# reazon-research/ReazonSpeech

Measured on AMD Instinct MI355X. Metric: RTFx (audio-sec/wall-sec), FastConformer-RNNT 619M batch=256, higher is better.
Workload: dtype bf16

## Files before the change

### reazonspeech_amd/csrc/k_gemm_bf16.hip

```cpp
#include <stdlib.h>

#include <atomic>

#include "rs_common.h"

namespace {

struct GemmParams {
    const uint16_t* A; const uint16_t* W; void* out;
    const float* bias; const float* residual; const int32_t* mask_lens;
    int lda, ldw, ldc, M, N, K, flags;
    float alpha;
    int mask_rows_per_step, mask_steps;
    int mask_row0;
    int tiles_m, tiles_n;
    int group_m;
    const float* res_ln_stats;
    const float* res_ln_g;
    const float* res_ln_b;
    uint16_t* out2;
    int ld2;
    int pairs;
    long long* trace;
    int cv_T2, cv_F2;
    unsigned cv_b_bytes, cv_t_bytes, cv_f_bytes;
    unsigned cv_seg_bytes;
    int cv_tps, cv_inv;
    const uint16_t* Wfm;
};

enum { OUT_BF16 = 0, OUT_F32 = 1, OUT_RES = 2, OUT_GLU = 3, OUT_RESLN = 4, OUT_BF16S = 5, OUT_F32S = 6, OUT_RES2 = 7 };

template <int N>
__device__ __forceinline__ void wait_vmcnt() {
    if constexpr (N == 0) asm volatile("s_waitcnt vmcnt(0)" ::: "memory");
    else if constexpr (N == 1) asm volatile("s_waitcnt vmcnt(1)" ::: "memory");
    else if constexpr (N == 2) asm volatile("s_waitcnt vmcnt(2)" ::: "memory");
    else if constexpr (N == 3) asm volatile("s_waitcnt vmcnt(3)" ::: "memory");
    else if constexpr (N == 4) asm volatile("s_waitcnt vmcnt(4)" ::: "memory");
    else if constexpr (N == 5) asm volatile("s_waitcnt vmcnt(5)" ::: "memory");
    else if constexpr (N == 6) asm volatile("s_waitcnt vmcnt(6)" ::: "memory");
    else if constexpr (N == 7) asm volatile("s_waitcnt vmcnt(7)" ::: "memory");
    else if constexpr (N == 8) asm volatile("s_waitcnt vmcnt(8)" ::: "memory");
    else if constexpr (N == 12) asm volatile("s_waitcnt vmcnt(12)" ::: "memory");
    else static_assert(N < 0, "add the vmcnt literal");
}

__device__ __forceinline__ void glds16(unsigned voff, const void* sbase, unsigned lds_dst) {
    asm volatile("s_mov_b32 m0, %2\n\ts_nop 0\n\tglobal_load_lds_dwordx4 %0, %1" :: "v"(voff), "s"(sbase), "s"(lds_dst) : "memory");
}

typedef unsigned u32x4_t __attribute__((ext_vector_type(4)));

__device__ __forceinline__ void gload16(u32x4_t& dst, unsigned voff, const void* sbase) {
    asm volatile("global_load_dwordx4 %0, %1, %2" : "=&v"(dst) : "v"(voff), "s"(sbase) : "memory");
}
__device__ __forceinline__ void breg_fence(u32x4_t (&r)[4]) {
    asm volatile("" : "+v"(r[0]), "+v"(r[1]), "+v"(r[2]), "+v"(r[3]) :: "memory");
}
template <int N>
__device__ __forceinline__ void wait_vmcnt_imm() {
    static_assert(N >= 0 && N < 64, "vmcnt is a 6-bit counter");
    asm volatile("s_waitcnt vmcnt(%0)" :: "n"(N) : "memory");
}

__global__ __launch_bounds__(256) void wfm_shuffle_kernel(const uint16_t* __restrict__ W, int ldw, int N, int K, uint16_t* __restrict__ out) {
    const size_t idx = (size_t)blockIdx.x * 256 + threadIdx.x;
    const size_t total = (size_t)N * K / 8;
    if (idx >= total) return;
    const int l = (int)(idx & 63);
    const size_t f = idx >> 6;
    const int kbs = K / 32;
    const int kb = (int)(f % kbs), nb = (int)(f / kbs);
    reinterpret_cast<uint4*>(out)[idx] = *reinterpret_cast<const uint4*>(W + (size_t)(nb * 16 + (l & 15)) * ldw + kb * 32 + (l >> 4) * 8);
}

__device__ __forceinline__ int swz64(int row) { return (row >> 1) & 7; }

__host__ __device__ inline void xcd_split(int xcount, int pair_mode, int& n_pairs, int& n_singles) {
    if (!pair_mode) { n_pairs = 0; n_singles = xcount; return; }
    const int rem = xcount % 64;
    n_singles = rem <= 32 ? rem : (xcount & 1);
    n_pairs = (xcount - n_singles) / 2;
}

template <int MI, int NI, int OUT_KIND, bool MASK, int PF>
__device__ __forceinline__ void smf16_epilogue(const GemmParams& p, f32x4_t (&acc)[MI][NI], char* scr, int cm0, int cn0,
                                               int wm, int wn, int lane) {
    constexpr bool SWOOSH = OUT_KIND == OUT_BF16S || OUT_KIND == OUT_F32S, RES2 = OUT_KIND == OUT_RES2;
    constexpr int OUT = OUT_KIND == OUT_BF16S ? OUT_BF16 : (OUT_KIND == OUT_F32S ? OUT_F32 : (RES2 ? OUT_RES : OUT_KIND));
    constexpr bool RESLN = OUT == OUT_RESLN, RES = OUT == OUT_RES || RESLN, out_f32 = OUT == OUT_F32 || RES, GLU = OUT == OUT_GLU, rowmask = MASK;
    constexpr int TM = MI * 16, TN = NI * 16;
    constexpr unsigned OOB = 0xfffffff0u;
    const int frow = lane & 15, fch = lane >> 4;
    const int flags = p.flags;
    const bool has_bias = flags & RS_GEMM_BIAS, relu = flags & RS_GEMM_RELU, silu = flags & RS_GEMM_SILU;
    const bool swl = SWOOSH && (flags & RS_GEMM_SWOOSHL), swr = SWOOSH && (flags & RS_GEMM_SWOOSHR);
    const float alpha = p.alpha;
    const size_t out_bytes = (size_t)p.M * p.ldc * (out_f32 ? 4 : 2);
    const auto out_rsrc = __builtin_amdgcn_make_buffer_rsrc(p.out, 0, (int)out_bytes, 0x00020000);
    const auto res_rsrc = __builtin_amdgcn_make_buffer_rsrc(const_cast<float*>(RES ? p.residual : (const float*)p.out), 0,
                                                            (int)out_bytes, 0x00020000);
    const auto bias_rsrc = __builtin_amdgcn_make_buffer_rsrc(const_cast<float*>(has_bias ? p.bias : (const float*)p.out), 0,
                                                             has_bias ? p.N * 4 : 0, 0x00020000);
    const int wrow0 = cm0 + wm * TM, wcol0 = cn0 + wn * TN;
    float4 bias_r[NI];
#pragma unroll
    for (int jj = 0; jj < NI; ++jj) {
        const int n = wcol0 + jj * 16 + 4 * fch;
        const u32x4_t b = __builtin_amdgcn_raw_buffer_load_b128(bias_rsrc, (unsigned)n * 4u, 0, 0);
        bias_r[jj] = __builtin_bit_cast(float4, b);
    }
    auto finish = [&](int i, int jj) -> float4 {
        float4 v = make_float4(acc[i][jj][0] + bias_r[jj].x, acc[i][jj][1] + bias_r[jj].y, acc[i][jj][2] + bias_r[jj].z,
                               acc[i][jj][3] + bias_r[jj].w);
        if (relu) { v.x = fmaxf(v.x, 0.f); v.y = fmaxf(v.y, 0.f); v.z = fmaxf(v.z, 0.f); v.w = fmaxf(v.w, 0.f); }
        if (silu) { v.x = silu_f(v.x); v.y = silu_f(v.y); v.z = silu_f(v.z); v.w = silu_f(v.w); }
        if constexpr (SWOOSH) {
            if (swl) { v.x = swoosh_l_f(v.x); v.y = swoosh_l_f(v.y); v.z = swoosh_l_f(v.z); v.w = swoosh_l_f(v.w); }
            if (swr) { v.x = swoosh_r_f(v.x); v.y = swoosh_r_f(v.y); v.z = swoosh_r_f(v.z); v.w = swoosh_r_f(v.w); }
        }
        v.x *= alpha; v.y *= alpha; v.z *= alpha; v.w *= alpha;
        return v;
    };
    auto row_keep = [&](int m) -> bool {
        if (!rowmask || m >= p.M) return true;
        const int step = (m + p.mask_row0) / p.mask_rows_per_step;
        const int b = step / p.mask_steps;
        return step - b * p.mask_steps < p.mask_lens[b];
    };
    if constexpr (GLU) {
        static_assert(NI == 4, "GLU epilogue: 64-column wave tiles");
        const int rr4 = lane >> 2, cc = lane & 3;
        const int ocol0 = wcol0 >> 1;
#pragma unroll
        for (int c = 0; c < MI / 2; ++c) {
#pragma unroll
            for (int il = 0; il < 2; ++il)
#pragma unroll
                for (int jj = 0; jj < 2; ++jj) {
                    const float4 a = finish(2 * c + il, jj), g = finish(2 * c + il, jj + 2);
                    const int row = il * 16 + frow;
                    const int piece = (jj * 2 + (fch >> 1)) ^ ((row >> 1) & 3);
                    *reinterpret_cast<u16x4_t*>(scr + row * 64 + piece * 16 + (fch & 1) * 8) =
                        pack_bf16x4(a.x * sigmoid_f(g.x), a.y * sigmoid_f(g.y), a.z * sigmoid_f(g.z), a.w * sigmoid_f(g.w));
                }
#pragma unroll
            for (int sgm = 0; sgm < 2; ++sgm) {
                const int row = sgm * 16 + rr4;
                u32x4_t d = *reinterpret_cast<const u32x4_t*>(scr + row * 64 + ((cc ^ ((row >> 1) & 3)) * 16));
                const int m = wrow0 + c * 32 + row, n = ocol0 + cc * 8;
                if (!row_keep(m)) d = (u32x4_t){0u, 0u, 0u, 0u};
                const unsigned off = (m < p.M && 2 * n < p.N) ? ((unsigned)m * (unsigned)p.ldc + (unsigned)n) * 2u : OOB;
                __builtin_amdgcn_raw_buffer_store_b128(d, out_rsrc, off, 0, 0);
            }
        }
    } else if constexpr (!out_f32) {
        const int rr8 = lane >> 3, cc = lane & 7;
#pragma unroll
        for (int c = 0; c < MI / 2; ++c) {
#pragma unroll
            for (int il = 0; il < 2; ++il)
#pragma unroll
                for (int jj = 0; jj < NI; ++jj) {
                    const float4 v = finish(2 * c + il, jj);
                    const int row = il * 16 + frow;
                    const int piece = (jj * 2 + (fch >> 1)) ^ (row & 7);
                    *reinterpret_cast<u16x4_t*>(scr + row * 128 + piece * 16 + (fch & 1) * 8) = pack_bf16x4(v.x, v.y, v.z, v.w);
                }
#pragma unroll
            for (int sgm = 0; sgm < 4; ++sgm) {
                const int row = sgm * 8 + rr8;
                u32x4_t d = *reinterpret_cast<const u32x4_t*>(scr + row * 128 + ((cc ^ (row & 7)) * 16));
                const int m = wrow0 + c * 32 + row, n = wcol0 + cc * 8;
                if (!row_keep(m)) d = (u32x4_t){0u, 0u, 0u, 0u};
                const unsigned off = (m < p.M && n < p.N) ? ((unsigned)m * (unsigned)p.ldc + (unsigned)n) * 2u : OOB;
                __builtin_amdgcn_raw_buffer_store_b128(d, out_rsrc, off, 0, 0);
            }
        }
    } else {
        const int rr4 = lane >> 4, cc = lane & 15;
        constexpr int PFE = (RESLN && MI >= 8 && PF > 1) ? PF - 1 : PF;
        constexpr int NPF = RES ? (PFE < 1 ? 1 : (PFE > MI ? MI : PFE)) : 1;
        u32x4_t rvq[NPF][4];
        float2 stq[NPF][4];
        float4 ln_g = make_float4(0.f, 0.f, 0.f, 0.f), ln_b = ln_g;
        const auto st_rsrc = __builtin_amdgcn_make_buffer_rsrc(const_cast<float*>(RESLN ? p.res_ln_stats : (const float*)p.out), 0,
                                                               RESLN ? p.M * 8 : 0, 0x00020000);
        if constexpr (RESLN) {
            const int n = wcol0 + cc * 4;
            if (n < p.N) {
                ln_g = *reinterpret_cast<const float4*>(p.res_ln_g + n);
                ln_b = *reinterpret_cast<const float4*>(p.res_ln_b + n);
            }
        }
        auto load_res = [&](int i, u32x4_t (&rv)[4], float2 (&st)[4]) {
#pragma unroll
            for (int sgm = 0; sgm < 4; ++sgm) {
                const int m = wrow0 + i * 16 + sgm * 4 + rr4, n = wcol0 + cc * 4;
                const unsigned off = (m < p.M && n < p.N) ? ((unsigned)m * (unsigned)p.ldc + (unsigned)n) * 4u : OOB;
                rv[sgm] = __builtin_amdgcn_raw_buffer_load_b128(res_rsrc, off, 0, 0);
                if constexpr (RESLN)
                    st[sgm] = __builtin_bit_cast(float2, __builtin_amdgcn_raw_buffer_load_b64(st_rsrc, m < p.M ? (unsigned)m * 8u : OOB, 0, 0));
            }
        };
        if constexpr (RES) {
#pragma unroll
            for (int d = 0; d < NPF; ++d) load_res(d, rvq[d], stq[d]);
            __builtin_amdgcn_sched_barrier(0);
        }
#pragma unroll
        for (int i = 0; i < MI; ++i) {
            u32x4_t rv[4];
            float2 st[4];
            if constexpr (RES) {
#pragma unroll
                for (int sgm = 0; sgm < 4; ++sgm) { rv[sgm] = rvq[i % NPF][sgm]; st[sgm] = stq[i % NPF][sgm]; }
            }
#pragma unroll
            for (int jj = 0; jj < NI; ++jj) {
                const float4 v = finish(i, jj);
                const int piece = (jj * 4 + fch) ^ frow;
                *reinterpret_cast<float4*>(scr + frow * 256 + piece * 16) = v;
            }
#pragma unroll
            for (int sgm = 0; sgm < 4; ++sgm) {
                const int row = sgm * 4 + rr4;
                float4 v = *reinterpret_cast<const float4*>(scr + row * 256 + ((cc ^ row) * 16));
                if constexpr (RES) {
                    float4 r = __builtin_bit_cast(float4, rv[sgm]);
                    if constexpr (RESLN) {
                        const float mean = st[sgm].x, rstd = st[sgm].y;
                        r.x = fmaf((r.x - mean) * rstd, ln_g.x, ln_b.x); r.y = fmaf((r.y - mean) * rstd, ln_g.y, ln_b.y);
                        r.z = fmaf((r.z - mean) * rstd, ln_g.z, ln_b.z); r.w = fmaf((r.w - mean) * rstd, ln_g.w, ln_b.w);
                    }
                    v.x += r.x; v.y += r.y; v.z += r.z; v.w += r.w;
                }
                const int m = wrow0 + i * 16 + row, n = wcol0 + cc * 4;
                if (!row_keep(m)) v = make_float4(0.f, 0.f, 0.f, 0.f);
                const unsigned off = (m < p.M && n < p.N) ? ((unsigned)m * (unsigned)p.ldc + (unsigned)n) * 4u : OOB;
                __builtin_amdgcn_raw_buffer_store_b128(__builtin_bit_cast(u32x4_t, v), out_rsrc, off, 0, 0);
                if constexpr (RES2) {
                    if (m < p.M && n < p.N) *reinterpret_cast<u16x4_t*>(p.out2 + (size_t)m * p.ld2 + n) = pack_bf16x4(v.x, v.y, v.z, v.w);
                }
            }
            if constexpr (RES) {
                if (i + NPF < MI) load_res(i + NPF, rvq[i % NPF], stq[i % NPF]);
            }
            __builtin_amdgcn_sched_barrier(0);
        }
    }
}

template <int BM, int OUT, bool MASK, int EPF, bool TRACE, bool CONVA = false, bool BREG = false>
__global__ __launch_bounds__(512, 2) void gemm_smf16_kernel(GemmParams p) {
    constexpr int BN = 256, WN = 4, NWAVES = 8;
    constexpr int TM = BM / 2, TN = BN / WN, MI = TM / 16, NI = TN / 16;
    constexpr int SLOT = 32768, NSLOT = 5;
    constexpr int LA = BM / 8 / NWAVES, LB = BN / 8 / NWAVES;
    constexpr int NPH = 2;
    static_assert((BM == 256 || BM == 192 || BM == 128 || BM == 64) && LB == 4 && (MI % 2) == 0 && BM * 128 <= SLOT, "tile heights");
    constexpr int A_BYTES = BM * 128, STAGE = A_BYTES + SLOT;
    constexpr bool R3 = 3 * STAGE <= NSLOT * SLOT;
    static_assert(!BREG || (!R3 && !TRACE && NI == 4), "BREG: split-ring tiles (256 / 192 rows) only");
    long long tr_t0 = 0, tr_t1 = 0, tr_t2 = 0, tr_w0 = 0, tr_stall = 0;
    if constexpr (TRACE) { tr_t0 = __builtin_readcyclecounter(); tr_w0 = (long long)wall_clock64(); }
    extern __shared__ __attribute__((aligned(16))) char smem[];
    const int tid = threadIdx.x, lane = tid & 63;
    const int wave = __builtin_amdgcn_readfirstlane(tid >> 6);
    const int wm = wave / WN, wn = wave % WN;
    const int frow = lane & 15, fch = lane >> 4;
    const unsigned lds0 = (unsigned)(size_t)(__attribute__((address_space(3))) char*)smem;

    const int nwg = p.tiles_m * p.tiles_n;
    const int bid = blockIdx.x;
    const int xcd = bid & 7, xslot = bid >> 3;
    const int q8 = nwg >> 3, rr = nwg & 7;
    const int xbase = xcd < rr ? xcd * (q8 + 1) : rr * (q8 + 1) + (xcd - rr) * q8;
    const int xcount = xcd < rr ? q8 + 1 : q8;
    int n_pairs, n_singles;
    xcd_split(xcount, p.pairs, n_pairs, n_singles);
    if (xslot >= n_pairs + n_singles) return;
    const int first_tile = xslot < n_pairs ? 2 * xslot : 2 * n_pairs + (xslot - n_pairs);
    const int n_my = xslot < n_pairs ? 2 : 1;
    const int nk = p.K / 64;
    const bool carry = p.pairs == 2 && nk >= 2;
    const int dr = lane >> 3, dpc = lane & 7;
    auto tile_origin = [&](int j, int& m0, int& n0) {
        const int wg = xbase + first_tile + j;
        const int per_group = p.group_m * p.tiles_n;
        const int g = wg / per_group, r = wg - g * per_group;
        const int left = p.tiles_m - g * p.group_m;
        const int gm = left < p.group_m ? left : p.group_m;
        const int tile_n = r / gm;
        m0 = (g * p.group_m + (r - tile_n * gm)) * BM;
        n0 = tile_n * BN;
    };
    auto lane_offsets = [&](int m0, int n0, unsigned (&o)[LA + LB]) {
#pragma unroll
        for (int j = 0; j < LA; ++j) {
            const int row = (wave + NWAVES * j) * 8 + dr;
            int gr = m0 + row;
            gr = gr < p.M ? gr : p.M - 1;
            if constexpr (CONVA) {
                const int bt = gr / p.cv_F2, f2 = gr - bt * p.cv_F2;
                const int b = bt / p.cv_T2, t2 = bt - b * p.cv_T2;
                o[j] = (unsigned)b * p.cv_b_bytes + (unsigned)t2 * p.cv_t_bytes + (unsigned)f2 * p.cv_f_bytes + (unsigned)((dpc ^ swz64(row)) * 16);
            } else {
                o[j] = (unsigned)gr * (unsigned)(p.lda * 2) + (unsigned)((dpc ^ swz64(row)) * 16);
            }
        }
        if constexpr (BREG) return;
#pragma unroll
        for (int j = 0; j < LB; ++j) {
            const int row = (wave * LB + j) * 8 + dr;
            int gr = n0 + row;
            gr = gr < p.N ? gr : p.N - 1;
            o[LA + j] = (unsigned)gr * (unsigned)(p.ldw * 2) + (unsigned)((dpc ^ swz64(row)) * 16);
        }
    };
    u32x4_t breg[2][4];
    const unsigned bvoff = (unsigned)lane * 16u;
    auto bfrag_base = [&](int n0_, int kb) -> const char* {
        const int nb = (n0_ >> 4) + wn * NI;
        const size_t off = ((size_t)nb * (size_t)(p.K >> 5) + (size_t)kb) << 10;
        return reinterpret_cast<const char*>(p.Wfm) + off;
    };
    auto bload = [&](int set, int n0_, int kb) {
        const char* b0 = bfrag_base(n0_, kb);
        const size_t jstride = (size_t)(p.K >> 5) << 10;
#pragma unroll
        for (int jj = 0; jj < 4; ++jj) gload16(breg[set][jj], bvoff, b0 + jj * jstride);
    };
    auto frag = [&](const char* part, int row, int chunk) -> bf16x8_t {
        return *reinterpret_cast<const bf16x8_t*>(part + row * 128 + ((chunk ^ swz64(row)) << 4));
    };
    auto wrap = [](int v) { return v >= NSLOT ? v - NSLOT : v; };

    int m0, n0;
    unsigned off[LA + LB], offn[LA + LB];
    tile_origin(0, m0, n0);
    lane_offsets(m0, n0, off);
    int sa = 0;
  for (int it = 0; it < n_my; ++it) {
    const bool has_next = carry && it + 1 < n_my;
    int m1 = m0, n1 = n0;
    if (has_next) { tile_origin(it + 1, m1, n1); lane_offsets(m1, n1, offn); }
    auto dma_a = [&](int j, int k, int dst) {
        const bool nx = k >= nk;
        const int kt = nx ? k - nk : k;
        size_t kbytes = (size_t)kt * 128;
        if constexpr (CONVA) {
            const int sg = (kt * p.cv_inv) >> 16;
            kbytes = (size_t)sg * p.cv_seg_bytes + (size_t)(kt - sg * p.cv_tps) * 128;
        }
        glds16(nx ? offn[j] : off[j], reinterpret_cast<const char*>(p.A) + kbytes, lds0 + dst + (wave + NWAVES * j) * 1024);
    };
    auto dma_b = [&](int j, int k, int dst) {
        if constexpr (BREG) return;
        const bool nx = k >= nk;
        glds16(nx ? offn[LA + j] : off[LA + j], reinterpret_cast<const char*>(p.W) + (size_t)(nx ? k - nk : k) * 128,
               lds0 + dst + (wave * LB + j) * 1024);
    };
    if constexpr (BREG) {
        if (it == 0 || !carry) {
            sa = 0;
#pragma unroll
            for (int j = 0; j < LA; ++j) dma_a(j, 0, 0);
            if (nk > 1) {
#pragma unroll
                for (int j = 0; j < LA; ++j) dma_a(j, 1, 2 * SLOT);
            }
            bload(0, n0, 0);
            bload(1, n0, 1);
            if (nk > 1) wait_vmcnt_imm<LA + 2 * NI>();
            else wait_vmcnt_imm<2 * NI>();
            __builtin_amdgcn_s_barrier();
        } else {
            bload(0, n0, 0);
            bload(1, n0, 1);
        }
    } else
    if (it == 0 || !carry) {
        sa = 0;
#pragma unroll
        for (int j = 0; j < LA; ++j) dma_a(j, 0, 0);
#pragma unroll
        for (int j = 0; j < LB; ++j) dma_b(j, 0, R3 ? A_BYTES : SLOT);
        if (nk > 1) {
#pragma unroll
            for (int j = 0; j < LA; ++j) dma_a(j, 1, R3 ? STAGE : 2 * SLOT);
            if constexpr (R3) {
#pragma unroll
                for (int j = 0; j < LB; ++j) dma_b(j, 1, STAGE + A_BYTES);
                wait_vmcnt<LA + LB>();
            } else if (wm == 1) {
#pragma unroll
                for (int j = 0; j < LB; ++j) dma_b(j, 1, 3 * SLOT);
                wait_vmcnt<LA + LB>();
            } else {
                wait_vmcnt<LA>();
            }
        } else {
            wait_vmcnt<0>();
        }
        __builtin_amdgcn_s_barrier();
    }
    if (wm == 1) __builtin_amdgcn_s_barrier();
    if constexpr (TRACE) tr_t1 = __builtin_readcyclecounter();

    f32x4_t acc[MI][NI];
#pragma unroll
    for (int i = 0; i < MI; ++i)
#pragma unroll
        for (int jj = 0; jj < NI; ++jj)
#pragma unroll
            for (int e = 0; e < 4; ++e) acc[i][jj][e] = 0.0f;

    for (int t = 0; t < nk; ++t) {
        auto wrap3 = [](int v) { return v >= 3 ? v - 3 : v; };
        const int a_cur = R3 ? sa * STAGE : sa * SLOT;
        const int b_cur = R3 ? a_cur + A_BYTES : wrap(sa + 1) * SLOT;
        const int bdst = R3 ? wrap3(sa + 2) * STAGE + A_BYTES : wrap(sa + 3) * SLOT;
        const int adst = R3 ? wrap3(sa + 2) * STAGE : wrap(sa + 4) * SLOT;
        constexpr int KB = R3 ? 2 : 1;
        const char* at = smem + a_cur;
        const char* bt = smem + b_cur;
        const bool has_1 = t + 1 < nk || has_next;
        const bool has_b = t + KB < nk || has_next, has_a = t + 2 < nk || has_next;
        auto wait_next = [&]() {
            if constexpr (R3) {
                if (has_a) wait_vmcnt<LA + LB>();
                else wait_vmcnt<0>();
            } else {
                if (has_a) wait_vmcnt<LA>();
                else wait_vmcnt<0>();
            }
        };
        auto timed_wait_next = [&]() {
            if constexpr (TRACE) { const long long a = __builtin_readcyclecounter(); wait_next(); tr_stall += __builtin_readcyclecounter() - a; }
            else wait_next();
        };
#pragma unroll
        for (int ks = 0; ks < NPH; ++ks) {
            const bool last = ks == NPH - 1;
            bf16x8_t bfr[NI], af[MI];
            const bool has_b1 = t + 1 < nk;
            if constexpr (!BREG) {
#pragma unroll
                for (int jj = 0; jj < NI; ++jj) bfr[jj] = frag(bt, wn * TN + jj * 16 + frow, ks * 4 + fch);
            }
#pragma unroll
            for (int i = 0; i < MI; ++i) af[i] = frag(at, wm * TM + i * 16 + frow, ks * 4 + fch);
            if constexpr (BREG) {
                if (ks == 0) wait_vmcnt_imm<NI>();
                else if (has_a && has_b1) wait_vmcnt_imm<LA + NI>();
                else if (has_a) wait_vmcnt_imm<LA>();
                else if (has_b1) wait_vmcnt_imm<NI>();
                else wait_vmcnt_imm<0>();
                breg_fence(breg[ks]);
#pragma unroll
                for (int jj = 0; jj < NI; ++jj) bfr[jj] = __builtin_bit_cast(bf16x8_t, breg[ks][jj]);
            }
            if (ks == 0 && has_b && (R3 || wm == 0)) {
                __builtin_amdgcn_sched_barrier(0);
#pragma unroll
                for (int j = 0; j < LB; ++j) dma_b(j, t + KB, bdst);
            }
            if constexpr (!BREG)
            if (last && has_1 && wm == 1) timed_wait_next();
            asm volatile("s_waitcnt lgkmcnt(0)" ::: "memory");
            __builtin_amdgcn_sched_barrier(0);
            __builtin_amdgcn_s_barrier();
            __builtin_amdgcn_sched_barrier(0);
            __builtin_amdgcn_s_setprio(1);
#pragma unroll
            for (int i = 0; i < MI; ++i) {
#pragma unroll
                for (int jj = 0; jj < NI; ++jj)
                    acc[i][jj] = __builtin_amdgcn_mfma_f32_16x16x32_bf16(bfr[jj], af[i], acc[i][jj], 0, 0, 0);
                if (ks == 0 && i < LA && has_a) {
                    __builtin_amdgcn_sched_barrier(0);
                    dma_a(i, t + 2, adst);
                    __builtin_amdgcn_sched_barrier(0);
                }
                if constexpr (!R3) {
                    if (ks == 1 && i < LB && wm == 1 && has_a) {
                        __builtin_amdgcn_sched_barrier(0);
                        dma_b(i, t + 2, a_cur);
                        __builtin_amdgcn_sched_barrier(0);
                    }
                }
            }
            if constexpr (BREG) {
                if (has_b1) {
                    __builtin_amdgcn_sched_barrier(0);
                    bload(ks, n0, 2 * (t + 1) + ks);
                    __builtin_amdgcn_sched_barrier(0);
                }
            } else
            if (last && has_1 && wm == 0) timed_wait_next();
            __builtin_amdgcn_s_setprio(0);
            __builtin_amdgcn_sched_barrier(0);
            __builtin_amdgcn_s_barrier();
            __builtin_amdgcn_sched_barrier(0);
        }
        sa = R3 ? wrap3(sa + 1) : wrap(sa + 2);
    }
    if (wm == 0) __builtin_amdgcn_s_barrier();
    {
        int em0 = __builtin_amdgcn_readfirstlane(m0), en0 = __builtin_amdgcn_readfirstlane(n0);
        asm volatile("" : "+s"(em0), "+s"(en0));
        if constexpr (TRACE) tr_t2 = __builtin_readcyclecounter();
        char* scr = smem + (R3 ? (sa + 2 >= 3 ? sa - 1 : sa + 2) * STAGE : wrap(sa + 4) * SLOT) + wave * 4096;
        smf16_epilogue<MI, NI, OUT, MASK, EPF>(p, acc, scr, em0, en0, wm, wn, lane);
        if constexpr (TRACE) {
            const long long t3 = __builtin_readcyclecounter();
            asm volatile("s_waitcnt vmcnt(0)" ::: "memory");
            const long long t4 = __builtin_readcyclecounter();
            if (lane == 0 && wn == 0) {
                long long* tr = p.trace + ((size_t)(xbase + first_tile + it) * 2 + wm) * 8;
                tr[0] = tr_t1 - tr_t0; tr[1] = tr_t2 - tr_t1; tr[2] = t3 - tr_t2; tr[3] = t4 - t3; tr[4] = tr_stall;
                tr[5] = bid; tr[6] = tr_w0; tr[7] = (long long)wall_clock64();
            }
            tr_t0 = __builtin_readcyclecounter(); tr_w0 = (long long)wall_clock64(); tr_stall = 0;
        }
    }
    if (it + 1 < n_my) {
        asm volatile("s_waitcnt lgkmcnt(0)" ::: "memory");
        __builtin_amdgcn_s_barrier();
        if (has_next) {
            m0 = m1; n0 = n1;
#pragma unroll
            for (int j = 0; j < LA + LB; ++j) off[j] = offn[j];
        } else {
            tile_origin(it + 1, m0, n0);
            lane_offsets(m0, n0, off);
        }
    }
  }
}

std::atomic<long long*> g_trace{nullptr};

int wfm_operand(rs_ctx* ctx, const uint16_t* W, int ldw, int N, int K, hipStream_t s, const uint16_t** out) {
    const size_t bytes = (size_t)N * K * 2;
    auto it = ctx->wfm.find(W);
    if (it != ctx->wfm.end()) { *out = reinterpret_cast<const uint16_t*>(it->second); return RS_OK; }
    bool registered = false;
    for (const auto& kv : ctx->tensors)
        if (kv.second.first == (const void*)W && kv.second.second >= (size_t)N * ldw * 2) { registered = true; break; }
    void* dst = nullptr;
    if (registered) {
        if (hipMalloc(&dst, bytes) != hipSuccess) return rs_fail(ctx, RS_EHIP, "gemm: no memory for the fragment-major copy of a weight (%zu bytes)", bytes);
        ctx->wfm[W] = dst;
    } else {
        if (ctx->wfm_scratch_bytes < bytes) {
            if (ctx->wfm_scratch) { (void)hipStreamSynchronize(s); (void)hipFree(ctx->wfm_scratch); ctx->wfm_scratch = nullptr; ctx->wfm_scratch_bytes = 0; }
            if (hipMalloc(&ctx->wfm_scratch, bytes) != hipSuccess) return rs_fail(ctx, RS_EHIP, "gemm: no memory for the fragment-major scratch (%zu bytes)", bytes);
            ctx->wfm_scratch_bytes = bytes;
        }
        dst = ctx->wfm_scratch;
    }
    const size_t pieces = (size_t)N * K / 8;
    hipLaunchKernelGGL(wfm_shuffle_kernel, dim3((unsigned)((pieces + 255) / 256)), dim3(256), 0, s, W, ldw, N, K, reinterpret_cast<uint16_t*>(dst));
    *out = reinterpret_cast<const uint16_t*>(dst);
    return RS_OK;
}

template <int BM>
int launch_smf16(rs_ctx* ctx, GemmParams& p, hipStream_t s) {
    constexpr int LDS = 5 * 32768;
    constexpr int EPF = 3;
    p.tiles_m = (p.M + BM - 1) / BM;
    p.tiles_n = (p.N + 255) / 256;
    const int ntiles = p.tiles_m * p.tiles_n;
    p.pairs = p.trace ? 0 : rs_knob(RS_KNOB_GEMM_PAIRS);
    int nwg;
    {
        int np, ns;
        xcd_split((ntiles + 7) / 8, p.pairs, np, ns);
        nwg = 8 * (np + ns);
        if (ntiles % 8 && ntiles > 8) {
            int np2, ns2;
            xcd_split(ntiles / 8, p.pairs, np2, ns2);
            if (8 * (np2 + ns2) > nwg) nwg = 8 * (np2 + ns2);
        }
    }
    const int group_m = rs_knob(RS_KNOB_GEMM_GROUP_M);
    p.group_m = group_m > 0 ? group_m
              : (p.tiles_n == 4 ? (p.K >= 4096 ? 2 : 6) : (p.K >= 4096 ? 4 : (p.tiles_n <= 8 && p.K <= 2560 ? 16 : 8)));
    const bool swoosh = p.flags & (RS_GEMM_SWOOSHL | RS_GEMM_SWOOSHR);
    const int out = (p.flags & RS_GEMM_RESIDUAL) ? (p.res_ln_stats ? OUT_RESLN : (p.out2 ? OUT_RES2 : OUT_RES))
                  : ((p.flags & RS_GEMM_OUT_F32) ? (swoosh ? OUT_F32S : OUT_F32) : ((p.flags & RS_GEMM_GLU) ? OUT_GLU : (swoosh ? OUT_BF16S : OUT_BF16)));
    const bool mask = p.flags & RS_GEMM_ROWMASK;
    if (p.cv_tps > 0) {
        if (int rc = rs_ensure_dynamic_lds(ctx, (const void*)gemm_smf16_kernel<BM, OUT_BF16, true, EPF, false, true>, LDS); rc != RS_OK) return rc;
        hipLaunchKernelGGL((gemm_smf16_kernel<BM, OUT_BF16, true, EPF, false, true>), dim3(nwg), dim3(512), LDS, s, p);
        return RS_OK;
    }
    if constexpr (BM >= 192) {
        if (rs_knob(RS_KNOB_GEMM_BREG) > 0 && !p.trace && !mask && p.N % 64 == 0 && p.N >= 256 &&
            (out == OUT_BF16 || out == OUT_RES || out == OUT_RESLN || out == OUT_F32 || out == OUT_GLU)) {
            if (int rc = wfm_operand(ctx, p.W, p.ldw, p.N, p.K, s, &p.Wfm); rc != RS_OK) return rc;
#define RS_SMF_B(O)                                                                                                \
            do {                                                                                                   \
                if (int rc = rs_ensure_dynamic_lds(ctx, (const void*)gemm_smf16_kernel<BM, O, false, EPF, false, false, true>, LDS); rc != RS_OK) return rc; \
                hipLaunchKernelGGL((gemm_smf16_kernel<BM, O, false, EPF, false, false, true>), dim3(nwg), dim3(512), LDS, s, p); \
            } while (0)
            if (out == OUT_BF16) RS_SMF_B(OUT_BF16);
            else if (out == OUT_RES) RS_SMF_B(OUT_RES);
            else if (out == OUT_RESLN) RS_SMF_B(OUT_RESLN);
            else if (out == OUT_F32) RS_SMF_B(OUT_F32);
            else RS_SMF_B(OUT_GLU);
#undef RS_SMF_B
            return RS_OK;
        }
    }
#define RS_SMF(O, MK, TR)                                                                                          \
    do {                                                                                                           \
        if (int rc = rs_ensure_dynamic_lds(ctx, (const void*)gemm_smf16_kernel<BM, O, MK, EPF, TR>, LDS); rc != RS_OK) return rc; \
        hipLaunchKernelGGL((gemm_smf16_kernel<BM, O, MK, EPF, TR>), dim3(nwg), dim3(512), LDS, s, p);  \
    } while (0)
    if (p.trace) {
        if constexpr (BM >= 192) {
            if (out == OUT_RES && !mask) RS_SMF(OUT_RES, false, true);
            else if (out == OUT_BF16 && !mask) RS_SMF(OUT_BF16, false, true);
            else return rs_fail(ctx, RS_EINVAL, "gemm trace: plain bf16 or residual output only");
            return RS_OK;
        } else {
            return rs_fail(ctx, RS_EINVAL, "gemm trace: 256- / 192-row tiles only");
        }
    }
    if (out == OUT_RES && !mask) RS_SMF(OUT_RES, false, false);
    else if (out == OUT_RESLN && !mask) RS_SMF(OUT_RESLN, false, false);
    else if (out == OUT_F32 && !mask) RS_SMF(OUT_F32, false, false);
    else if (out == OUT_BF16 && !mask) RS_SMF(OUT_BF16, false, false);
    else if (out == OUT_BF16 && mask) RS_SMF(OUT_BF16, true, false);
    else if (out == OUT_GLU && !mask) RS_SMF(OUT_GLU, false, false);
    else if (out == OUT_RES2 && !mask) RS_SMF(OUT_RES2, false, false);
    else if (out == OUT_BF16S && !mask) RS_SMF(OUT_BF16S, false, false);
    else if (out == OUT_F32S && !mask) RS_SMF(OUT_F32S, false, false);
    else return rs_fail(ctx, RS_EINVAL, "gemm: the row mask combines with plain bf16 output only");
#undef RS_SMF
    return RS_OK;
}

int pick_tile_height(int M, int N, int K, int n_cus, int flags) {
    static const int bms[4] = {256, 192, 128, 64};
    static const double kt[4] = {1.246, 1.146, 1.03, 0.96}, fix[4] = {11.5, 7.0, 5.0, 4.0};
    const long tn = (N + 255) / 256;
    const int nk = K / 64;
    const double epi = (flags & RS_GEMM_RESIDUAL) ? 13.0 : ((flags & RS_GEMM_OUT_F32) ? 6.5 : 0.0);
    int best = 256;
    double best_cost = 1e30;
    for (int i = 0; i < 4; ++i) {
        const long tiles = (long)((M + bms[i] - 1) / bms[i]) * tn;
        const long rounds = (tiles + n_cus - 1) / n_cus;
        const double cost = (double)rounds * (nk * kt[i] + fix[i] + epi * bms[i] / 192.0);
        if (cost < best_cost) { best_cost = cost; best = bms[i]; }
    }
    return best;
}

}

extern "C" void rs_debug_set_gemm_tile(int bm) { rs_knob_set(RS_KNOB_GEMM_TILE, bm); }
extern "C" void rs_debug_set_gemm_trace(long long* buf) { g_trace = buf; }
extern "C" void rs_debug_set_gemm_group_m(int v) { rs_knob_set(RS_KNOB_GEMM_GROUP_M, v); }
extern "C" void rs_debug_set_gemm_pairs(int v) { rs_knob_set(RS_KNOB_GEMM_PAIRS, v); }
extern "C" void rs_debug_set_gemm_breg(int v) { rs_knob_set(RS_KNOB_GEMM_BREG, v); }
extern "C" int rs_debug_gemm_tile_height(int M, int N, int K, int n_cus, int flags) { return pick_tile_height(M, N, K, n_cus > 0 ? n_cus : 256, flags); }

static int launch_rows(rs_ctx* ctx, GemmParams& p, int bm, hipStream_t s) {
    switch (bm) {
        case 256: return launch_smf16<256>(ctx, p, s);
        case 192: return launch_smf16<192>(ctx, p, s);
        case 128: return launch_smf16<128>(ctx, p, s);
        case 64: return launch_smf16<64>(ctx, p, s);
        default: return rs_fail(ctx, RS_EINVAL, "gemm: tile height %d (256, 192, 128 or 64)", bm);
    }
}

int rs_launch_gemm(rs_ctx* ctx, const rs_gemm_args& a, hipStream_t s) {
    if (a.M <= 0 || a.N <= 0 || a.K <= 0) return rs_fail(ctx, RS_EINVAL, "gemm: empty shape %d %d %d", a.M, a.N, a.K);
    if (a.K % 64) return rs_fail(ctx, RS_EINVAL, "gemm: K=%d must be a multiple of 64", a.K);
    const bool f32 = a.flags & (RS_GEMM_OUT_F32 | RS_GEMM_RESIDUAL);
    if (a.N % 4 || a.ldc % 4) return rs_fail(ctx, RS_EINVAL, "gemm: N=%d and ldc=%d must be multiples of 4", a.N, a.ldc);
    if (!f32 && ((a.ldc % 8) || (a.N % 8))) return rs_fail(ctx, RS_EINVAL, "gemm: bf16 output needs N %% 8 == 0 and ldc %% 8 == 0 (got %d, %d)", a.N, a.ldc);
    if ((a.lda % 8) || (a.ldw % 8) || ((uintptr_t)a.A & 15) || ((uintptr_t)a.W & 15) || ((uintptr_t)a.out & 15))
        return rs_fail(ctx, RS_EINVAL, "gemm: operands must be 16-byte aligned (lda %d ldw %d)", a.lda, a.ldw);
    if ((a.flags & RS_GEMM_ROWMASK) && (!a.mask_lens || a.mask_rows_per_step <= 0 || a.mask_steps <= 0))
        return rs_fail(ctx, RS_EINVAL, "gemm: row mask requested without lens");
    if ((a.flags & RS_GEMM_ROWMASK) && f32) return rs_fail(ctx, RS_EINVAL, "gemm: the row mask combines with bf16 output only");
    if ((a.flags & RS_GEMM_BIAS) && (!a.bias || ((uintptr_t)a.bias & 15)))
        return rs_fail(ctx, RS_EINVAL, "gemm: bias flag without a 16-byte aligned pointer");
    if ((a.flags & RS_GEMM_RESIDUAL) && (!a.residual || ((uintptr_t)a.residual & 15)))
        return rs_fail(ctx, RS_EINVAL, "gemm: residual flag without a 16-byte aligned pointer");
    if (a.res_ln_stats && (!(a.flags & RS_GEMM_RESIDUAL) || !a.res_ln_g || !a.res_ln_b || ((uintptr_t)a.res_ln_g & 15) ||
                           ((uintptr_t)a.res_ln_b & 15) || ((uintptr_t)a.res_ln_stats & 7)))
        return rs_fail(ctx, RS_EINVAL, "gemm: a normalised residual needs the residual flag, row statistics and aligned weight / bias");
    if (a.flags & RS_GEMM_GLU) {
        if (a.flags & (RS_GEMM_RELU | RS_GEMM_SILU | RS_GEMM_RESIDUAL | RS_GEMM_OUT_F32 | RS_GEMM_ROWMASK | RS_GEMM_SWOOSHL | RS_GEMM_SWOOSHR))
            return rs_fail(ctx, RS_EINVAL, "gemm: GLU combines with a bias only");
        if ((a.N % 64) || a.alpha != 1.0f) return rs_fail(ctx, RS_EINVAL, "gemm: GLU needs N %% 64 == 0 and alpha == 1 (N=%d)", a.N);
    }
    if (a.out_bf16 && (!(a.flags & RS_GEMM_RESIDUAL) || a.res_ln_stats || (a.ld_bf16 % 4) || ((uintptr_t)a.out_bf16 & 7)))
        return rs_fail(ctx, RS_EINVAL, "gemm: the bf16 copy combines with a plain residual output only (8-byte aligned, pitch %% 4)");
    if ((a.flags & (RS_GEMM_SWOOSHL | RS_GEMM_SWOOSHR)) && (a.flags & RS_GEMM_RESIDUAL))
        return rs_fail(ctx, RS_EINVAL, "gemm: the Swoosh activations combine with plain bf16 / f32 output only");
    if ((size_t)a.N * a.ldw * 2 >= (1ull << 32)) return rs_fail(ctx, RS_EINVAL, "gemm: weight matrix beyond 4 GiB");
    int cv_tps = 0, cv_inv = 0;
    if (a.conv_C > 0) {
        const int C = a.conv_C;
        if (C % 64 || a.K != 9 * C || a.conv_T2 <= 0 || a.conv_F2 <= 0 || a.M % (a.conv_T2 * a.conv_F2) || 2 * (a.conv_T2 - 1) + 3 > a.conv_T1 ||
            2 * (a.conv_F2 - 1) + 3 > a.conv_F1)
            return rs_fail(ctx, RS_EINVAL, "gemm: convolution patches need C %% 64 == 0, K == 9 C and an input that covers the output (C %d K %d)", C, a.K);
        if ((a.flags & ~(RS_GEMM_BIAS | RS_GEMM_RELU | RS_GEMM_SILU)) != RS_GEMM_ROWMASK)
            return rs_fail(ctx, RS_EINVAL, "gemm: convolution patches combine with plain bf16 output and the row mask only");
        if ((size_t)(a.M / (a.conv_T2 * a.conv_F2)) * a.conv_T1 * a.conv_F1 * C * 2 >= (1ull << 32) - 65536)
            return rs_fail(ctx, RS_EINVAL, "gemm: convolution input beyond 4 GiB (run it in chunks of utterances)");
        cv_tps = 3 * C / 64;
        cv_inv = (65536 + cv_tps - 1) / cv_tps;
        for (int k = 0; k < 2 * (a.K / 64); ++k)
            if (((k * cv_inv) >> 16) != k / cv_tps) return rs_fail(ctx, RS_EINVAL, "gemm: K-tile reciprocal is not exact for C = %d", C);
    }
    const int tile = rs_knob(RS_KNOB_GEMM_TILE);
    const int bm = tile > 0 ? tile : pick_tile_height(a.M, a.N, a.K, rs_n_cus(ctx), a.flags);
    if (bm != 256 && bm != 192 && bm != 128 && bm != 64) return rs_fail(ctx, RS_EINVAL, "gemm: RS_GEMM_TILE=%d (256, 192, 128 or 64)", bm);
    const size_t out_row = (size_t)a.ldc * (f32 ? 4 : 2), a_row = a.conv_C > 0 ? 2 : (size_t)a.lda * 2;
    size_t max_rows = ((1ull << 31) - 65536) / out_row;
    if (((1ull << 32) - 65536) / a_row < max_rows) max_rows = ((1ull << 32) - 65536) / a_row;
    if (a.conv_C > 0 && (size_t)a.M > max_rows / 768 * 768) return rs_fail(ctx, RS_EINVAL, "gemm: convolution output beyond 2 GiB (run it in chunks of utterances)");
    if (max_rows < 768) return rs_fail(ctx, RS_EINVAL, "gemm: row pitch too large (lda %d, ldc %d)", a.lda, a.ldc);
    max_rows = max_rows / 768 * 768;
    const double flops = 2.0 * a.M * (double)a.N * a.K;
    const double bytes = 2.0 * ((double)a.M * a.K + (double)a.N * a.K) +
                         (double)a.M * a.N * ((a.flags & RS_GEMM_OUT_F32) ? 4 : ((a.flags & RS_GEMM_GLU) ? 1 : 2)) +
                         ((a.flags & RS_GEMM_RESIDUAL) ? (double)a.M * a.N * 4 : 0.0);
    ctx->prof_tag[0] = a.M; ctx->prof_tag[1] = a.N; ctx->prof_tag[2] = a.K; ctx->prof_tag[3] = a.flags;
    rs_prof_scope prof(ctx, RS_PROF_GEMM, s, flops, bytes);
    for (size_t r0 = 0; r0 < (size_t)a.M; r0 += max_rows) {
        GemmParams p;
        const size_t rows = (size_t)a.M - r0 < max_rows ? (size_t)a.M - r0 : max_rows;
        p.A = a.A + r0 * a.lda; p.W = a.W;
        p.out = reinterpret_cast<char*>(a.out) + r0 * out_row;
        p.bias = a.bias; p.residual = a.residual ? a.residual + r0 * a.ldc : nullptr; p.mask_lens = a.mask_lens;
        p.res_ln_stats = a.res_ln_stats ? a.res_ln_stats + r0 * 2 : nullptr; p.res_ln_g = a.res_ln_g; p.res_ln_b = a.res_ln_b;
        p.lda = a.lda; p.ldw = a.ldw; p.ldc = a.ldc; p.M = (int)rows; p.N = a.N; p.K = a.K; p.flags = a.flags;
        p.alpha = a.alpha; p.mask_rows_per_step = a.mask_rows_per_step; p.mask_steps = a.mask_steps; p.mask_row0 = (int)r0;
        p.out2 = a.out_bf16 ? a.out_bf16 + r0 * a.ld_bf16 : nullptr; p.ld2 = a.ld_bf16;
        p.tiles_m = p.tiles_n = 0; p.group_m = 1;
        p.trace = g_trace.load();
        p.cv_tps = cv_tps; p.cv_inv = cv_inv; p.cv_T2 = a.conv_T2; p.cv_F2 = a.conv_F2;
        p.Wfm = nullptr;
        if (cv_tps > 0) {
            p.trace = nullptr;
            p.cv_b_bytes = (unsigned)((size_t)a.conv_T1 * a.conv_F1 * a.conv_C * 2);
            p.cv_t_bytes = (unsigned)((size_t)2 * a.conv_F1 * a.conv_C * 2);
            p.cv_f_bytes = (unsigned)(2 * a.conv_C * 2);
            p.cv_seg_bytes = (unsigned)((size_t)a.conv_F1 * a.conv_C * 2);
        }
        if (int rc = launch_rows(ctx, p, bm, s); rc != RS_OK) return rc;
    }
    prof.end();
    RS_CHECK_LAUNCH(ctx, "gemm_smf16");
    return RS_OK;
}
```

### reazonspeech_amd/csrc/rs_knobs.h

```cpp
#pragma once
#include <stdlib.h>
#include <string.h>

#include <atomic>
#include <mutex>

#include "../../include/rs_asr.h"

#define RS_KNOBS(X)                                                                                                                   \
    X(GEMM_TILE, "RS_GEMM_TILE", INT, 0, "forced GEMM tile height (256 / 192 / 128 / 64); 0 = by shape")                              \
    X(GEMM_GROUP_M, "RS_GEMM_GROUP_M", INT, 0, "row panels per XCD tile group; 0 = by shape")                                         \
    X(GEMM_PAIRS, "RS_GEMM_PAIRS", INT, 2, "2 = two tiles per workgroup, LDS ring carried over; 1 = ring restarted; 0 = one tile")    \
    X(GEMM_BREG, "RS_GEMM_BREG", INT, 0, "1 = 256- / 192-row launches keep the weight operand out of LDS (global -> VGPR)")           \
    X(ATTN_PERSIST, "RS_ATTN_PERSIST", INT, 0, "1 = full attention on resident workgroups that walk the items (n >= 2: on n)")        \
    X(ATTN_STREAM, "RS_ATTN_STREAM", INT, 0, "1 = the streaming attention form (+ 16 x mask: phases left out, for timing)")           \
    X(ATTN64, "RS_ATTN64", INT, 4, "head_dim 64: key blocks per chunk; 0 = the one-workgroup-per-CU geometry")                        \
    X(ATTN64_NW, "RS_ATTN64_NW", INT, 4, "head_dim 64: waves per workgroup (the second number of $RS_ATTN64)")                        \
    X(ATTN_F32_OLD, "RS_ATTN_F32_OLD", PRESENT, 0, "float32 attention: the first form (one wave per key sum)")                        \
    X(ATTN_F32_KEYS, "RS_ATTN_F32_KEYS", PRESENT, 0, "float32 attention: the second form (keys over lanes, no MFMA)")                 \
    X(GLU_GENERIC, "RS_GLU_GENERIC", INT, 0, "GLU + depthwise conv: 1 = the any-kernel-size path, 2 = the f32-tile kernel on the gated layout") \
    X(SUB_IM2COL, "RS_SUB_IM2COL", PRESENT, 0, "ESPnet subsampling: gather the 3 x 3 patches into a matrix first (sizes the workspace too)") \
    X(FUSE_GLU, "RS_FUSE_GLU", INT, 1, "context default: 0 = GLU in the depthwise kernel, not the pw1 GEMM epilogue")                 \
    X(DEFER_OUT_NORM, "RS_DEFER_OUT_NORM", INT, 1, "context default: 0 = every output norm stores its f32 rows")                      \
    X(DECODE_SCREEN, "RS_DECODE_SCREEN", INT, 1, "context default: 0 = exact evaluation of every joint column")                       \
    X(DECODE_NARROW, "RS_DECODE_NARROW", INT, 1, "context default: 0 = the wide-tile LSTM / projection kernels")                      \
    X(DECODE_NO_XCD, "RS_DECODE_NO_XCD", PRESENT, 0, "greedy decode: joint grids not padded to a multiple of 8 column tiles")         \
    X(DECODE_NO_LOOKAHEAD, "RS_DECODE_NO_LOOKAHEAD", PRESENT, 0, "greedy decode: one frame per utterance and step at every batch size") \
    X(VERIFY_WIDE, "RS_VERIFY_WIDE", INT, 0, "screened joint: 1 = a workgroup per row for V <= 3072 too")                             \
    X(DECODE_TRACE, "RS_DECODE_TRACE", PRESENT, 0, "greedy decode: print the step count of every call to stderr")                     \
    X(BEAM_SPEC, "RS_BEAM_SPEC", INT, 3, "beam search: evaluations asked for per iteration (1 .. 8; sizes the workspace too)")         \
    X(BEAM_TRACE, "RS_BEAM_TRACE", PRESENT, 0, "beam search: phase timing of the step kernel")                                        \
    X(BEAM_RECORD_LDS, "RS_BEAM_RECORD_LDS", PRESENT, 0, "beam search: the any-vocabulary record kernel on a small vocabulary")       \
    X(AVSR_POSCONV_OLD, "RS_AVSR_POSCONV_OLD", PRESENT, 0, "AV-HuBERT positional convolution: the VALU form")                         \
    X(K2_CONV1_OLD, "RS_K2_CONV1_OLD", PRESENT, 0, "Zipformer conv1: the VALU form (the one other channel counts run)")               \
    X(K2_ATTW_SWEEPS, "RS_K2_ATTW_SWEEPS", INT, 1, "Zipformer attention weights: 3 = the three-sweep kernel")                         \
    X(K2_CONV2_FUSED, "RS_K2_CONV2_FUSED", INT, 1, "default of option k2_conv2_fused: 0 = patch matrix + GEMM launch")                \
    X(K2_CNX_FUSED, "RS_K2_CNX_FUSED", INT, 1, "default of option k2_cnx_fused: 0 = the ConvNeXt pointwise pair as two GEMM launches")

enum rs_knob_id {
#define RS_KNOB_ENUM(id, env, kind, def, what) RS_KNOB_##id,
    RS_KNOBS(RS_KNOB_ENUM)
#undef RS_KNOB_ENUM
    RS_KNOB_COUNT
};
enum rs_knob_kind { RS_KNOB_PRESENT, RS_KNOB_INT };
struct rs_knob_row { const char* env; rs_knob_kind kind; int def; };
static const rs_knob_row rs_knob_rows[RS_KNOB_COUNT] = {
#define RS_KNOB_ROW(id, env, kind, def, what) {env, RS_KNOB_##kind, def},
    RS_KNOBS(RS_KNOB_ROW)
#undef RS_KNOB_ROW
};

struct rs_knob_table {
    std::atomic<int> value[RS_KNOB_COUNT];
    std::atomic<bool> given[RS_KNOB_COUNT];
    std::once_flag once;
};
inline rs_knob_table rs_knob_state;

inline void rs_knobs_read_env() {
    std::call_once(rs_knob_state.once, [] {
        rs_knob_table& t = rs_knob_state;
        for (int i = 0; i < RS_KNOB_COUNT; ++i) { t.value[i] = rs_knob_rows[i].def; t.given[i] = false; }
        for (int i = 0; i < RS_KNOB_COUNT; ++i) {
            const char* e = i == RS_KNOB_ATTN64_NW ? nullptr : getenv(rs_knob_rows[i].env);
            if (!e) continue;
            t.given[i] = true;
            t.value[i] = rs_knob_rows[i].kind == RS_KNOB_PRESENT ? 1 : atoi(e);
            if (i == RS_KNOB_ATTN64) {
                t.given[RS_KNOB_ATTN64_NW] = true;
                if (const char* c = strchr(e, ',')) t.value[RS_KNOB_ATTN64_NW] = atoi(c + 1);
            }
        }
    });
}

inline int rs_knob(rs_knob_id id) { rs_knobs_read_env(); return rs_knob_state.value[id].load(std::memory_order_relaxed); }
inline bool rs_knob_given(rs_knob_id id) { rs_knobs_read_env(); return rs_knob_state.given[id].load(std::memory_order_relaxed); }
inline void rs_knob_set(rs_knob_id id, int v) { rs_knobs_read_env(); rs_knob_state.value[id].store(v, std::memory_order_relaxed); }

inline int rs_knob_find(const char* env_name) {
    for (int i = 0; env_name && i < RS_KNOB_COUNT; ++i)
        if (!strcmp(env_name, rs_knob_rows[i].env)) return i;
    return -1;
}
inline int rs_knob_set_named(const char* env_name, int v) {
    const int i = rs_knob_find(env_name);
    if (i < 0) return RS_EINVAL;
    rs_knob_set((rs_knob_id)i, v);
    return RS_OK;
}
inline int rs_knob_get_named(const char* env_name, int* v) {
    const int i = rs_knob_find(env_name);
    if (i < 0 || !v) return RS_EINVAL;
    *v = rs_knob((rs_knob_id)i);
    return RS_OK;
}
```

Measured before the change: 46100.

## Add XCD-aware tile cost model and optional two-launch GEMM row split

Replaces the simple rounds estimate in the tile-height picker with a model that counts rounds per XCD, including the two-tiles-per-workgroup pairing. Adds an opt-in planner that splits a GEMM into two launches. The first covers full rounds at one tile height and the second covers the partial last round at a smaller height, with plans cached per shape. The split is meant to cut tail-round idle time at the cost of an extra launch. It is off by default, but the revised cost model changes the default tile choice.

After: 46010. No clear change (-0.2%).

```diff
diff --git a/reazonspeech_amd/csrc/k_gemm_bf16.hip b/reazonspeech_amd/csrc/k_gemm_bf16.hip
--- a/reazonspeech_amd/csrc/k_gemm_bf16.hip
+++ b/reazonspeech_amd/csrc/k_gemm_bf16.hip
@@ -1,6 +1,7 @@
 #include <stdlib.h>
 
 #include <atomic>
+#include <mutex>
 
 #include "rs_common.h"
 
@@ -646,21 +647,118 @@
     return RS_OK;
 }
 
+const int tile_heights[4] = {256, 192, 128, 64};
+
+double tile_time(int i, int K, int flags) {
+    static const double kt[4] = {1.246, 1.146, 1.03, 0.96}, fix[4] = {11.5, 7.0, 5.0, 4.0};
+    const double epi = (flags & RS_GEMM_RESIDUAL) ? 13.0 : ((flags & RS_GEMM_OUT_F32) ? 6.5 : 0.0);
+    return (K / 64) * kt[i] + fix[i] + epi * tile_heights[i] / 192.0;
+}
+
+long xcd_rounds(long xcount, int cpx, int pair_mode) {
+    if (xcount <= 0) return 0;
+    int np, ns;
+    xcd_split((int)xcount, pair_mode, np, ns);
+    const long base = 2L * (np / cpx);
+    const int rp = np % cpx;
+    if (ns == 0) return base + (rp ? 2 : 0);
+    const long room = 2L * (cpx - rp);
+    if (ns <= room) return base + (rp || ns > cpx - rp ? 2 : 1);
+    return base + 2 + (ns - room + cpx - 1) / cpx;
+}
+long launch_rounds(long tiles, int n_cus, int pair_mode) {
+    const int cpx = n_cus >= 8 ? n_cus / 8 : 1;
+    const long hi = xcd_rounds((tiles + 7) / 8, cpx, pair_mode), lo = xcd_rounds(tiles / 8, cpx, pair_mode);
+    return hi > lo ? hi : lo;
+}
+double launch_cost(int M, int N, int K, int n_cus, int flags, int i, int pair_mode) {
+    const long tiles = (long)((M + tile_heights[i] - 1) / tile_heights[i]) * ((N + 255) / 256);
+    return (double)launch_rounds(tiles, n_cus, pair_mode) * tile_time(i, K, flags);
+}
+
 int pick_tile_height(int M, int N, int K, int n_cus, int flags) {
-    static const int bms[4] = {256, 192, 128, 64};
-    static const double kt[4] = {1.246, 1.146, 1.03, 0.96}, fix[4] = {11.5, 7.0, 5.0, 4.0};
-    const long tn = (N + 255) / 256;
-    const int nk = K / 64;
-    const double epi = (flags & RS_GEMM_RESIDUAL) ? 13.0 : ((flags & RS_GEMM_OUT_F32) ? 6.5 : 0.0);
+    const int pair_mode = rs_knob(RS_KNOB_GEMM_PAIRS);
     int best = 256;
     double best_cost = 1e30;
     for (int i = 0; i < 4; ++i) {
-        const long tiles = (long)((M + bms[i] - 1) / bms[i]) * tn;
-        const long rounds = (tiles + n_cus - 1) / n_cus;
-        const double cost = (double)rounds * (nk * kt[i] + fix[i] + epi * bms[i] / 192.0);
-        if (cost < best_cost) { best_cost = cost; best = bms[i]; }
+        const double cost = launch_cost(M, N, K, n_cus, flags, i, pair_mode);
+        if (cost < best_cost) { best_cost = cost; best = tile_heights[i]; }
     }
     return best;
+}
+
+constexpr double GEMM_PLAN_TAIL_US = 4.4;
+
+struct gemm_plan { int rows1, bm1, bm2; double cost, single_cost; };
+
+gemm_plan plan_search(int M, int N, int K, int n_cus, int flags, int pair_mode) {
+    gemm_plan best{0, 0, 256, 1e30, 0.0};
+    for (int i = 0; i < 4; ++i) {
+        const double c = launch_cost(M, N, K, n_cus, flags, i, pair_mode);
+        if (c < best.cost) { best.cost = c; best.bm2 = tile_heights[i]; }
+    }
+    const double single = best.single_cost = best.cost;
+    const long tn = (N + 255) / 256;
+    for (int i = 0; i < 4; ++i) {
+        const int bm1 = tile_heights[i];
+        const double t1 = tile_time(i, K, flags);
+        long last_rounds = -1;
+        for (long tm = (M - 1) / bm1; tm >= 1; --tm) {
+            const long r1 = launch_rounds(tm * tn, n_cus, pair_mode);
+            if (r1 == last_rounds) continue;
+            last_rounds = r1;
+            const double c1 = (double)r1 * t1 + GEMM_PLAN_TAIL_US;
+            if (c1 >= single) continue;
+            const int rest = M - (int)(tm * bm1);
+            for (int j = 0; j < 4; ++j) {
+                const double c = c1 + launch_cost(rest, N, K, n_cus, flags, j, pair_mode);
+                if (c < best.cost) best = gemm_plan{(int)(tm * bm1), bm1, tile_heights[j], c, single};
+            }
+        }
+    }
+    return best;
+}
+
+gemm_plan plan_rows(int M, int N, int K, int n_cus, int flags) {
+    struct entry { int M, N, K, n_cus, epi, pair_mode; gemm_plan plan; };
+    static std::mutex mu;
+    static entry cache[64];
+    static int n_cached = 0, next = 0;
+    const int epi = flags & (RS_GEMM_RESIDUAL | RS_GEMM_OUT_F32), pair_mode = rs_knob(RS_KNOB_GEMM_PAIRS);
+    {
+        std::lock_guard<std::mutex> lock(mu);
+        for (int i = 0; i < n_cached; ++i) {
+            const entry& e = cache[i];
+            if (e.M == M && e.N == N && e.K == K && e.n_cus == n_cus && e.epi == epi && e.pair_mode == pair_mode) return e.plan;
+        }
+    }
+    const gemm_plan plan = plan_search(M, N, K, n_cus, flags, pair_mode);
+    std::lock_guard<std::mutex> lock(mu);
+    cache[next] = entry{M, N, K, n_cus, epi, pair_mode, plan};
+    next = (next + 1) % 64;
+    if (n_cached < 64) ++n_cached;
+    return plan;
+}
+
+std::atomic<int> g_plan_rows1{0}, g_plan_bm1{0}, g_plan_bm2{0};
+
+bool tile_height_ok(int bm) { return bm == 256 || bm == 192 || bm == 128 || bm == 64; }
+
+bool plan_off() { return rs_knob(RS_KNOB_GEMM_TILE) > 0 || rs_knob(RS_KNOB_GEMM_PLAN) <= 0; }
+
+int plan_segments(int M, int N, int K, int n_cus, int flags, int seg[2][2]) {
+    seg[1][0] = seg[1][1] = 0;
+    seg[0][0] = M;
+    const int f_rows1 = g_plan_rows1.load(), f_bm1 = g_plan_bm1.load(), f_bm2 = g_plan_bm2.load();
+    if (f_rows1 > 0 && f_rows1 < M) {
+        if (!tile_height_ok(f_bm1) || !tile_height_ok(f_bm2) || f_rows1 % f_bm1) return 0;
+        seg[0][0] = f_rows1; seg[0][1] = f_bm1; seg[1][0] = M - f_rows1; seg[1][1] = f_bm2;
+        return 2;
+    }
+    const gemm_plan plan = plan_rows(M, N, K, n_cus, flags);
+    if (plan.rows1 == 0) { seg[0][1] = plan.bm2; return 1; }
+    seg[0][0] = plan.rows1; seg[0][1] = plan.bm1; seg[1][0] = M - plan.rows1; seg[1][1] = plan.bm2;
+    return 2;
 }
 
 }
@@ -671,6 +769,20 @@
 extern "C" void rs_debug_set_gemm_pairs(int v) { rs_knob_set(RS_KNOB_GEMM_PAIRS, v); }
 extern "C" void rs_debug_set_gemm_breg(int v) { rs_knob_set(RS_KNOB_GEMM_BREG, v); }
 extern "C" int rs_debug_gemm_tile_height(int M, int N, int K, int n_cus, int flags) { return pick_tile_height(M, N, K, n_cus > 0 ? n_cus : 256, flags); }
+extern "C" int rs_debug_gemm_plan(int M, int N, int K, int n_cus, int flags, int out[4]) {
+    int seg[2][2] = {{M, 0}, {0, 0}};
+    n_cus = n_cus > 0 ? n_cus : 256;
+    int n = 1;
+    if (plan_off()) seg[0][1] = rs_knob(RS_KNOB_GEMM_TILE) > 0 ? rs_knob(RS_KNOB_GEMM_TILE) : pick_tile_height(M, N, K, n_cus, flags);
+    else n = plan_segments(M, N, K, n_cus, flags, seg);
+    out[0] = seg[0][0]; out[1] = seg[0][1]; out[2] = seg[1][0]; out[3] = seg[1][1];
+    return n;
+}
+extern "C" void rs_debug_gemm_plan_cost(int M, int N, int K, int n_cus, int flags, double out[2]) {
+    const gemm_plan plan = plan_search(M, N, K, n_cus > 0 ? n_cus : 256, flags, rs_knob(RS_KNOB_GEMM_PAIRS));
+    out[0] = plan.cost; out[1] = plan.single_cost;
+}
+extern "C" void rs_debug_set_gemm_plan(int rows1, int bm1, int bm2) { g_plan_rows1 = 0; g_plan_bm1 = bm1; g_plan_bm2 = bm2; g_plan_rows1 = rows1; }
 
 static int launch_rows(rs_ctx* ctx, GemmParams& p, int bm, hipStream_t s) {
     switch (bm) {
@@ -740,9 +852,15 @@
                          ((a.flags & RS_GEMM_RESIDUAL) ? (double)a.M * a.N * 4 : 0.0);
     ctx->prof_tag[0] = a.M; ctx->prof_tag[1] = a.N; ctx->prof_tag[2] = a.K; ctx->prof_tag[3] = a.flags;
     rs_prof_scope prof(ctx, RS_PROF_GEMM, s, flops, bytes);
-    for (size_t r0 = 0; r0 < (size_t)a.M; r0 += max_rows) {
+    const bool planned = !plan_off() && a.conv_C <= 0 && !g_trace.load();
+    for (size_t c0 = 0; c0 < (size_t)a.M; c0 += max_rows) {
+      const size_t chunk = (size_t)a.M - c0 < max_rows ? (size_t)a.M - c0 : max_rows;
+      int seg[2][2] = {{(int)chunk, bm}, {0, 0}};
+      const int n_seg = planned ? plan_segments((int)chunk, a.N, a.K, rs_n_cus(ctx), a.flags, seg) : 1;
+      if (n_seg == 0) return rs_fail(ctx, RS_EINVAL, "gemm: forced plan %d rows at %d, the rest at %d", g_plan_rows1.load(), g_plan_bm1.load(), g_plan_bm2.load());
+      for (int si = 0; si < n_seg; ++si) {
         GemmParams p;
-        const size_t rows = (size_t)a.M - r0 < max_rows ? (size_t)a.M - r0 : max_rows;
+        const size_t r0 = c0 + (si ? (size_t)seg[0][0] : 0), rows = (size_t)seg[si][0];
         p.A = a.A + r0 * a.lda; p.W = a.W;
         p.out = reinterpret_cast<char*>(a.out) + r0 * out_row;
         p.bias = a.bias; p.residual = a.residual ? a.residual + r0 * a.ldc : nullptr; p.mask_lens = a.mask_lens;
@@ -761,9 +879,22 @@
             p.cv_f_bytes = (unsigned)(2 * a.conv_C * 2);
             p.cv_seg_bytes = (unsigned)((size_t)a.conv_F1 * a.conv_C * 2);
         }
-        if (int rc = launch_rows(ctx, p, bm, s); rc != RS_OK) return rc;
+        if (int rc = launch_rows(ctx, p, seg[si][1], s); rc != RS_OK) return rc;
+      }
     }
     prof.end();
     RS_CHECK_LAUNCH(ctx, "gemm_smf16");
     return RS_OK;
 }
+
+extern "C" int rs_debug_gemm_bf16_ex(rs_ctx* ctx, const uint16_t* A, int lda, const uint16_t* W, int ldw, void* out, int ldc, int M, int N, int K,
+                                     int flags, const float* bias, float alpha, const float* residual, const int32_t* mask_lens,
+                                     int mask_rows_per_step, int mask_steps, const float* res_ln_stats, const float* res_ln_g,
+                                     const float* res_ln_b, uint16_t* out_bf16, int ld_bf16, void* stream) {
+    if (!ctx) return RS_EINVAL;
+    if (!A || !W || !out) return rs_fail(ctx, RS_EINVAL, "gemm: null pointer");
+    rs_gemm_args g{A, lda, W, ldw, out, ldc, M, N, K, flags, bias, alpha, residual, mask_lens, mask_rows_per_step, mask_steps};
+    g.res_ln_stats = res_ln_stats; g.res_ln_g = res_ln_g; g.res_ln_b = res_ln_b;
+    g.out_bf16 = out_bf16; g.ld_bf16 = ld_bf16;
+    return rs_launch_gemm(ctx, g, (hipStream_t)stream);
+}
diff --git a/reazonspeech_amd/csrc/rs_knobs.h b/reazonspeech_amd/csrc/rs_knobs.h
--- a/reazonspeech_amd/csrc/rs_knobs.h
+++ b/reazonspeech_amd/csrc/rs_knobs.h
@@ -12,6 +12,7 @@
     X(GEMM_GROUP_M, "RS_GEMM_GROUP_M", INT, 0, "row panels per XCD tile group; 0 = by shape")                                         \
     X(GEMM_PAIRS, "RS_GEMM_PAIRS", INT, 2, "2 = two tiles per workgroup, LDS ring carried over; 1 = ring restarted; 0 = one tile")    \
     X(GEMM_BREG, "RS_GEMM_BREG", INT, 0, "1 = 256- / 192-row launches keep the weight operand out of LDS (global -> VGPR)")           \
+    X(GEMM_PLAN, "RS_GEMM_PLAN", INT, 0, "1 = a launch's partial last round may run as a second launch at a lower tile height; 0 = one height") \
     X(ATTN_PERSIST, "RS_ATTN_PERSIST", INT, 0, "1 = full attention on resident workgroups that walk the items (n >= 2: on n)")        \
     X(ATTN_STREAM, "RS_ATTN_STREAM", INT, 0, "1 = the streaming attention form (+ 16 x mask: phases left out, for timing)")           \
     X(ATTN64, "RS_ATTN64", INT, 4, "head_dim 64: key blocks per chunk; 0 = the one-workgroup-per-CU geometry")                        \
```
